# resibots/limbo

Measured on AMD Instinct MI355X. Metric: GP compute()+log_lik evaluations/sec at N=4096 D=6 fp64, higher is better.
Workload: dtype f64

## Files before the change

### limbo_amd/csrc/gemm.hip

```cpp
#include "dev.h"
#include <hip/hip_ext.h>
#include <cstdio>
#include <cstdint>
#include <cstdlib>
#include <map>
#include <mutex>
#include <tuple>
#include <vector>
#include <algorithm>

#ifdef GEMM_TIMING
__device__ long long g_gemm_ts[16];
#define GTS(i) do { if (threadIdx.x == 0 && blockIdx.x == 0 && lwg == (int)blockIdx.x) g_gemm_ts[i] = clock64(); } while (0)
__device__ long long g_gemm64_ts[24];
#define GTS64(i) do { if (threadIdx.x == 0 && blockIdx.x == 0 && lwg == (int)blockIdx.x) g_gemm64_ts[i] = clock64(); } while (0)
#else
#define GTS(i) do { } while (0)
#define GTS64(i) do { } while (0)
#endif
#ifdef GEMM_TIMING
#define GTS64_(i) GTS64(i)
#endif
#include "gemm_glds64.h"
#ifndef GEMM_ABL
#define GEMM_ABL 0
#endif


template <bool KMAJOR, int ROWS, int BK>
struct Stager {
    static constexpr int PER = ROWS * BK / 256;
    static constexpr int STRIDE = ROWS + 16;
    static constexpr int KSTR = BK + 2;
    static constexpr int ELEMS = KMAJOR ? ROWS * KSTR : BK * STRIDE;
    double r[PER];
    template <bool MASKK>
    __device__ __forceinline__ void load(const double* __restrict__ P, int64_t ld, int rl, int kl)
    {
        const int t = threadIdx.x;
        if (!KMAJOR) {
            const int i = t % ROWS, kk0 = t / ROWS;
            constexpr int KS = 256 / ROWS;
            const int ic = i < rl ? i : rl - 1;
#pragma unroll
            for (int q = 0; q < PER; ++q) {
                const int kk = kk0 + KS * q;
                const int kc = kk < kl ? kk : kl - 1;
                const double v = P[ic + (int64_t)kc * ld];
                r[q] = MASKK ? v * (kk < kl ? 1.0 : 0.0) : v;
            }
        }
        else {
            const int kk = t % BK, j0 = t / BK;
            constexpr int JS = 256 / BK;
            const int kc = kk < kl ? kk : kl - 1;
            const double km = kk < kl ? 1.0 : 0.0;
#pragma unroll
            for (int q = 0; q < PER; ++q) {
                const int j = j0 + JS * q;
                const int jc = j < rl ? j : rl - 1;
                const double v = P[kc + (int64_t)jc * ld];
                r[q] = MASKK ? v * km : v;
            }
        }
    }
    __device__ __forceinline__ void store(double* __restrict__ S) const
    {
        const int t = threadIdx.x;
        if (!KMAJOR) {
            const int i = t % ROWS, kk0 = t / ROWS;
            constexpr int KS = 256 / ROWS;
#pragma unroll
            for (int q = 0; q < PER; ++q)
                S[(kk0 + KS * q) * STRIDE + i] = r[q];
        }
        else {
            const int kk = t % BK, j0 = t / BK;
            constexpr int JS = 256 / BK;
#pragma unroll
            for (int q = 0; q < PER; ++q)
                S[(j0 + JS * q) * KSTR + kk] = r[q];
        }
    }
    static __device__ __forceinline__ double at(const double* __restrict__ S, int row, int kq)
    {
        if (!KMAJOR)
            return S[kq * STRIDE + row];
        else
            return S[row * KSTR + kq];
    }
};

template <int TM, int TN, int BKT, int NBUF, bool AK, bool BK, bool BATCH = false>
__global__ __launch_bounds__(256) void k_gemm4(GemmArgs g_)
{
    GemmArgs gb;
    if (BATCH) {
        gb = g_;
        gemm_rebase(gb);
    }
    const GemmArgs& g = BATCH ? gb : g_;
    using SA = Stager<AK, TM, BKT>;
    using SB = Stager<BK, TN, BKT>;
    constexpr int RA = TM / 2 / 16;
    constexpr int RB = TN / 2 / 4;
    __shared__ __attribute__((aligned(16))) double lds[NBUF][SA::ELEMS + SB::ELEMS];
    const int tiles_m = (int)((g.m + TM - 1) / TM);
    const int tiles_n = (int)((g.n + TN - 1) / TN);
    int wg = blockIdx.x;
    {
        const int nwg = gridDim.x;
        const int q = nwg / 8, r = nwg % 8, xcd = wg % 8, idx = wg / 8;
        wg = (xcd < r ? xcd * (q + 1) : r * (q + 1) + (xcd - r) * q) + idx;
    }
    int ti, tj;
    if (g.tri) {
        const int sc = wg / g.fold_len;
        int rr = wg % g.fold_len;
        const int t0 = first_live_tile<TM, TN>(g, sc), c0 = tiles_m - t0;
        if (rr < c0) {
            tj = sc;
            ti = t0 + rr;
        }
        else {
            tj = tiles_n - 1 - sc;
            const int t1 = first_live_tile<TM, TN>(g, tj);
            rr -= c0;
            if (tj == sc || rr >= tiles_m - t1)
                return;
            ti = t1 + rr;
        }
    }
    else {
        ti = wg % tiles_m;
        tj = wg / tiles_m;
    }
    const int64_t row0 = (int64_t)ti * TM, col0 = (int64_t)tj * TN;
    int64_t kbeg = 0;
    if (g.ktri) {
        kbeg = (row0 > col0 ? row0 : col0);
        kbeg -= kbeg % BKT;
    }
    const int64_t kend = g.k;

    const int lane = threadIdx.x & 63;
    const int wave = threadIdx.x >> 6;
    const int wm = (wave & 1) * (TM / 2), wn = (wave >> 1) * (TN / 2);
    const int arow = wm + (lane & 15);
    const int bcol = wn + (lane & 3);
    const int kq = lane >> 4;

    const double* Ap = AK ? g.A + kbeg + row0 * g.lda : g.A + row0 + kbeg * g.lda;
    const double* Bp = BK ? g.B + kbeg + col0 * g.ldb : g.B + col0 + kbeg * g.ldb;
    const int64_t a_kstep = AK ? (int64_t)BKT : (int64_t)BKT * g.lda;
    const int64_t b_kstep = BK ? (int64_t)BKT : (int64_t)BKT * g.ldb;
    const int64_t mrows = g.m - row0, ncols = g.n - col0;
    const int mr = (int)(mrows < TM ? mrows : TM), nc = (int)(ncols < TN ? ncols : TN);

    double acc[RA][RB];
#pragma unroll
    for (int a = 0; a < RA; ++a)
#pragma unroll
        for (int b = 0; b < RB; ++b)
            acc[a][b] = 0.0;

    using WT = WaveTileC<RA, RB>;
    double* Cw = g.C + (col0 + wn) * g.ldc + row0 + wm;
    const int rlim = mr - wm < WT::R ? mr - wm : WT::R, clim = nc - wn < WT::CN ? nc - wn : WT::CN;
    const bool live = rlim > 0 && clim > 0;
    constexpr bool CPRE = (NBUF == 1);
    double cv[WT::NIT];
    if (CPRE && live && g.overwrite != 1)
        WT::load(cv, Cw, g.ldc, rlim, clim, lane);

    SA sa;
    SB sb;
    int64_t kleft = kend - kbeg;
    if (kleft > 0) {
        const int kl = (int)(kleft < BKT ? kleft : BKT);
        sa.template load<true>(Ap, g.lda, mr, kl);
        sb.template load<false>(Bp, g.ldb, nc, kl);
        sa.store(lds[0]);
        sb.store(lds[0] + SA::ELEMS);
    }
    __syncthreads();
    int buf = 0;
    for (int64_t k0 = kbeg; k0 < kend; k0 += BKT) {
#if GEMM_ABL != 1
        const bool more = (NBUF == 2) && (k0 + BKT < kend);
#endif
#if GEMM_ABL == 1
        const bool more = false;
#endif
        if (more) {
            Ap += a_kstep;
            Bp += b_kstep;
            const int64_t kleft2 = kend - k0 - BKT;
            const int kl = (int)(kleft2 < BKT ? kleft2 : BKT);
            sa.template load<true>(Ap, g.lda, mr, kl);
            sb.template load<false>(Bp, g.ldb, nc, kl);
        }
        const double* As = lds[buf];
        const double* Bs = lds[buf] + SA::ELEMS;
#pragma unroll
        for (int ks = 0; ks < BKT; ks += 4) {
            double af[RA], bf[RB];
#pragma unroll
            for (int x = 0; x < RA; ++x)
                af[x] = SA::at(As, arow + 16 * x, ks + kq);
#pragma unroll
            for (int x = 0; x < RB; ++x)
                bf[x] = SB::at(Bs, bcol + 4 * x, ks + kq);
#pragma unroll
            for (int n = 0; n < RB; ++n)
#pragma unroll
                for (int m = 0; m < RA; ++m)
#if GEMM_ABL == 2
                    acc[m][n] += af[m] * bf[n] * (ks == 0 && m == 0 && n == 0 ? 1.0 : 0.0);
#else
                    acc[m][n] = mfma4(af[m], bf[n], acc[m][n]);
#endif
        }
        if (NBUF == 2) {
            if (more) {
                sa.store(lds[buf ^ 1]);
                sb.store(lds[buf ^ 1] + SA::ELEMS);
            }
            __syncthreads();
            buf ^= 1;
        }
    }

    static_assert(4 * WT::SCRATCH <= NBUF * (SA::ELEMS + SB::ELEMS), "transposition scratch must fit in the operand stages");
    if (!CPRE && live && g.overwrite != 1)
        WT::load(cv, Cw, g.ldc, rlim, clim, lane);
    if (NBUF == 1)
        __syncthreads();
    if (live)
        WT::store(acc, cv, &lds[0][0] + wave * WT::SCRATCH, Cw, g.ldc, rlim, clim, g.overwrite, lane);
}

template <typename K>
static void launch_k_named(const char* name, K kern_single, K kern_batched, dim3 grid, dim3 block, hipStream_t s, const GemmArgs& g0)
{
    GemmArgs g = g0;
    g.bt = g_batch.bt;
    grid.z = (unsigned)g_batch.G;
    K kern = g.bt ? kern_batched : kern_single;
    if (g.stop_event)
        GPE_LAUNCH_STOP(name, kern, grid, block, 0, s, (hipEvent_t)g.stop_event, g);
    else
        GPE_LAUNCH_NAMED(name, kern, grid, block, 0, s, g);
}
#define launch_k(ks, ...) launch_k_named(#ks, ks, __VA_ARGS__)
template <int TM, int TN, int BKT, int NBUF>
static void launch_tile(hipStream_t s, const GemmArgs& g0)
{
    GemmArgs g = g0;
    const int tiles_m = (int)((g.m + TM - 1) / TM), tiles_n = (int)((g.n + TN - 1) / TN);
    int64_t tiles = (int64_t)tiles_m * tiles_n;
    if (g.tri) {
        int fold = 1;
        const int nsup = (tiles_n + 1) / 2;
        for (int sc = 0; sc < nsup; ++sc) {
            const int t2 = tiles_n - 1 - sc;
            int len = tiles_m - first_live_tile<TM, TN>(g, sc);
            if (t2 != sc)
                len += tiles_m - first_live_tile<TM, TN>(g, t2);
            fold = len > fold ? len : fold;
        }
        g.fold_len = fold;
        tiles = (int64_t)nsup * fold;
    }
    dim3 grid((unsigned)tiles), block(256);
    if (!g.a_kmajor && !g.b_kmajor)
        launch_k(k_gemm4<TM, TN, BKT, NBUF, false, false>, k_gemm4<TM, TN, BKT, NBUF, false, false, true>, grid, block, s, g);
    else if (!g.a_kmajor && g.b_kmajor)
        launch_k(k_gemm4<TM, TN, BKT, NBUF, false, true>, k_gemm4<TM, TN, BKT, NBUF, false, true, true>, grid, block, s, g);
    else if (g.a_kmajor && !g.b_kmajor)
        launch_k(k_gemm4<TM, TN, BKT, NBUF, true, false>, k_gemm4<TM, TN, BKT, NBUF, true, false, true>, grid, block, s, g);
    else
        launch_k(k_gemm4<TM, TN, BKT, NBUF, true, true>, k_gemm4<TM, TN, BKT, NBUF, true, true, true>, grid, block, s, g);
}


template <int TM, int TN, int WM, int WN, int BKT, int NST, int EPC = 0, int MINB = 1, bool BATCH = false>
__global__ __launch_bounds__(WM* WN * 64, MINB) void k_gemm_glds(GemmArgs g_)
{
    GemmArgs gb;
    if (BATCH) {
        gb = g_;
        gemm_rebase(gb);
    }
    const GemmArgs& g = BATCH ? gb : g_;
    static_assert(TM == 128 && TN == 128, "one k-row of an operand tile = one 1 KiB glds instruction");
    constexpr int NWV = WM * WN;
    constexpr int SA = TM + 16, SB = TN + 16;
    constexpr int STAGE = BKT * (SA + SB);
    constexpr int RA = TM / WM / 16, RB = TN / WN / 4;
    constexpr int LPW = 2 * BKT / NWV;
    __shared__ __attribute__((aligned(16))) double lds[NST * STAGE];

    const int tiles_m = (int)((g.m + TM - 1) / TM);
    const int tiles_n = (int)((g.n + TN - 1) / TN);
    if (g.rhs_rows > 0)
        gemm_rhs_rows<64 * NWV, MINB == 1>(g, g.rhs_rows, (int)gridDim.x, lds);
    for (int lwg = blockIdx.x; lwg < g.total; lwg += gridDim.x) {
    int wg = lwg;
    {
        const int nwg = g.total;
        const int q = nwg / 8, r = nwg % 8, xcd = wg % 8, idx = wg / 8;
        wg = (xcd < r ? xcd * (q + 1) : r * (q + 1) + (xcd - r) * q) + idx;
    }
    int ti, tj;
    if (g.tile_map) {
        const int pk = g.tile_map[lwg];
        if (pk < 0)
            continue;
        ti = pk & 0xffff;
        tj = pk >> 16;
    }
    else if (g.tri) {
        const int sc = wg / g.fold_len;
        int rr = wg % g.fold_len;
        const int t0 = first_live_tile<TM, TN>(g, sc), c0 = tiles_m - t0;
        if (rr < c0) {
            tj = sc;
            ti = t0 + rr;
        }
        else {
            tj = tiles_n - 1 - sc;
            const int t1 = first_live_tile<TM, TN>(g, tj);
            rr -= c0;
            if (tj == sc || rr >= tiles_m - t1)
                continue;
            ti = t1 + rr;
        }
    }
    else {
        ti = wg % tiles_m;
        tj = wg / tiles_m;
    }
    const int64_t row0 = (int64_t)ti * TM, col0 = (int64_t)tj * TN;
    const int64_t mrows = g.m - row0, ncols = g.n - col0;
    const int mr = (int)(mrows < TM ? mrows : TM), nc = (int)(ncols < TN ? ncols : TN);

    const int lane = threadIdx.x & 63;
    const int wave = __builtin_amdgcn_readfirstlane(threadIdx.x >> 6);
    const int wm = (wave % WM) * (TM / WM), wn = (wave / WM) * (TN / WN);
    const int arow = wm + (lane & 15), bcol = wn + (lane & 3), kq = lane >> 4;

    int ra = 2 * lane, rb = 2 * lane;
    {
        const int ma = (mr - 1) & ~1, mb = (nc - 1) & ~1;
        ra = ra < ma ? ra : ma;
        rb = rb < mb ? rb : mb;
    }
    const int64_t kbeg = g.ktri ? (row0 > col0 ? row0 : col0) : 0;
    const double* pa = g.A + row0 + ra + ((int64_t)wave + kbeg) * g.lda;
    const double* pb = g.B + col0 + rb + ((int64_t)wave + kbeg) * g.ldb;
    const int64_t astep = (int64_t)NWV * g.lda, bstep = (int64_t)NWV * g.ldb;

    auto issue = [&](int stage) {
        double* sa = lds + stage * STAGE + wave * SA;
        double* sb = lds + stage * STAGE + BKT * SA + wave * SB;
#pragma unroll
        for (int q = 0; q < BKT / NWV; ++q) {
            __builtin_amdgcn_global_load_lds(pa, (lds_void_t*)(sa + q * NWV * SA), 16, 0, 0);
            __builtin_amdgcn_global_load_lds(pb, (lds_void_t*)(sb + q * NWV * SB), 16, 0, 0);
            pa += astep;
            pb += bstep;
        }
    };

    double acc[RA][RB];
#pragma unroll
    for (int a = 0; a < RA; ++a)
#pragma unroll
        for (int b = 0; b < RB; ++b)
            acc[a][b] = 0.0;

    const int nk = (int)((g.k - kbeg) / BKT);
    GTS(0);
    issue(0);
    for (int t = 0; t < nk; ++t) {
        const int st = t % NST;
        if (t + 1 < nk) {
            issue((t + 1) % NST);
            asm volatile("s_waitcnt vmcnt(%0)" ::"n"(LPW) : "memory");
        }
        else
            asm volatile("s_waitcnt vmcnt(0)" ::: "memory");
        __builtin_amdgcn_s_barrier();
        if (t == 0)
            GTS(1);
        if (t == 1)
            GTS(2);
        if (t == 2)
            GTS(3);
        const double* As = lds + st * STAGE;
        const double* Bs = As + BKT * SA;
#pragma unroll
        for (int ks = 0; ks < BKT; ks += 4) {
            double af[RA], bf[RB];
#pragma unroll
            for (int x = 0; x < RA; ++x)
                af[x] = As[(ks + kq) * SA + arow + 16 * x];
#pragma unroll
            for (int x = 0; x < RB; ++x)
                bf[x] = Bs[(ks + kq) * SB + bcol + 4 * x];
#pragma unroll
            for (int n = 0; n < RB; ++n)
#pragma unroll
                for (int m = 0; m < RA; ++m)
                    acc[m][n] = mfma4(af[m], bf[n], acc[m][n]);
        }
        if (t == 1)
            GTS(6);
        asm volatile("s_waitcnt lgkmcnt(0)" ::: "memory");
        __builtin_amdgcn_s_barrier();
        if (t == 1)
            GTS(7);
    }
    GTS(4);

    {
        using WT = WaveTileC<RA, RB>;
        constexpr int SCR = EPC > 0 ? WT::SCRATCH / EPC : WT::SCRATCH;
        static_assert(NWV * SCR <= NST * STAGE, "transposition scratch must fit in the operand stages");
        double* Cw = g.C + (col0 + wn) * g.ldc + row0 + wm;
        const int rlim = mr - wm < WT::R ? mr - wm : WT::R, clim = nc - wn < WT::CN ? nc - wn : WT::CN;
        if (rlim > 0 && clim > 0) {
            if constexpr (EPC > 0)
                WT::template rmw_chunked<EPC>(acc, lds + wave * SCR, Cw, g.ldc, rlim, clim, g.overwrite, lane);
            else {
                double cv[WT::NIT];
                if (g.overwrite != 1)
                    WT::load(cv, Cw, g.ldc, rlim, clim, lane);
                WT::store(acc, cv, lds + wave * WT::SCRATCH, Cw, g.ldc, rlim, clim, g.overwrite, lane);
            }
        }
    }
    __syncthreads();
    GTS(5);
    }
}
#ifdef GEMM_TIMING
void dump_gemm_timing()
{
    {
        long long q[24];
        (void)hipMemcpyFromSymbol(q, HIP_SYMBOL(g_gemm64_ts), sizeof(q));
        printf("k_gemm_glds64 WG0 first tile, cycles: start->k-tile 0 begins %lld | k-tiles:", q[1] - q[0]);
        for (int t = 1; t < 16; ++t)
            printf(" %lld", q[1 + t] - q[t]);
        printf(" %lld | epilogue %lld | total %lld\n", q[17] - q[16], q[18] - q[17], q[18] - q[0]);
    }
    long long h[16];
    (void)hipMemcpyFromSymbol(h, HIP_SYMBOL(g_gemm_ts), sizeof(h));
    printf("k_gemm_glds WG0 first tile, cycles: prologue (first stage landed) %lld | k-tile 0 %lld | k-tile 1 %lld (mfma part %lld, closing barrier %lld) | whole k loop %lld | epilogue %lld | total %lld\n",
           h[1] - h[0], h[2] - h[1], h[3] - h[2], h[6] - h[2], h[7] - h[6], h[4] - h[1], h[5] - h[4], h[5] - h[0]);
    printf("  epilogue: issue 32 loads %lld | loads complete %lld | issue 32 stores %lld | stores complete %lld | tail %lld\n", h[8] - h[4],
           h[9] - h[8], h[10] - h[9], h[11] - h[10], h[5] - h[11]);
}
#endif

template <int BKT, int NST, int MINB, int NWV, bool BATCH = false>
__global__ __launch_bounds__(64 * NWV, MINB) void k_gemm_glds64(GemmArgs g_)
{
    GemmArgs gb;
    if (BATCH) {
        gb = g_;
        gemm_rebase(gb);
    }
    const GemmArgs& g = BATCH ? gb : g_;
    __shared__ __attribute__((aligned(16))) double lds[NST * Glds64Shape<BKT>::STAGE];
    gemm_glds64_body<BKT, NST, NWV>(g, lds, (int)blockIdx.x, (int)gridDim.x, false);
}

static void launch_glds64(hipStream_t s, const GemmArgs& g0)
{
    constexpr int TM = 64, TN = 64;
    GemmArgs g = g0;
    const int tiles_m = (int)((g.m + TM - 1) / TM), tiles_n = (int)((g.n + TN - 1) / TN);
    int64_t tiles = (int64_t)tiles_m * tiles_n;
    if (g.tri) {
        int fold = 1;
        const int nsup = (tiles_n + 1) / 2;
        for (int sc = 0; sc < nsup; ++sc) {
            const int t2 = tiles_n - 1 - sc;
            int len = tiles_m - first_live_tile<TM, TN>(g, sc);
            if (t2 != sc)
                len += tiles_m - first_live_tile<TM, TN>(g, t2);
            fold = len > fold ? len : fold;
        }
        g.fold_len = fold;
        tiles = (int64_t)nsup * fold;
    }
    g.total = (int)tiles;
    if ((int64_t)g.total * g_batch.G > 256)
        launch_k(k_gemm_glds64<16, 4, 2, 4>, k_gemm_glds64<16, 4, 2, 4, true>, dim3((unsigned)tiles), dim3(256), s, g);
    else
        launch_k(k_gemm_glds64<16, 4, 1, 8>, k_gemm_glds64<16, 4, 1, 8, true>, dim3((unsigned)tiles), dim3(512), s, g);
}

static bool glds_ok(const GemmArgs& g)
{
    return !g.a_kmajor && !g.b_kmajor && !g.ktri && g.k >= 32 && g.k % 32 == 0 && (g.lda % 2) == 0 && (g.ldb % 2) == 0
        && ((uintptr_t)g.A % 16) == 0 && ((uintptr_t)g.B % 16) == 0;
}

#define TRI_BAND 8
struct TriMapKey {
    int dev, tiles_m, tiles_n;
    int64_t off;
    bool operator<(const TriMapKey& o) const
    {
        return std::tie(dev, tiles_m, tiles_n, off) < std::tie(o.dev, o.tiles_m, o.tiles_n, o.off);
    }
};
static int tri_tile_map_host(const GemmArgs& g, std::vector<int>& tab)
{
    constexpr int TM = 128, TN = 128;
    const int tiles_m = (int)((g.m + TM - 1) / TM), tiles_n = (int)((g.n + TN - 1) / TN);
    std::vector<int> first(tiles_n);
    for (int tj = 0; tj < tiles_n; ++tj)
        first[tj] = first_live_tile<TM, TN>(g, tj);
    std::vector<int> seq;
    for (int r0 = 0; r0 < tiles_m; r0 += TRI_BAND) {
        const int r1 = std::min(tiles_m, r0 + TRI_BAND);
        for (int tj = 0; tj < tiles_n; ++tj)
            for (int ti = std::max(r0, first[tj]); ti < r1; ++ti)
                seq.push_back(ti | (tj << 16));
    }
    const int T = (int)seq.size(), q = T / 8, r = T % 8, slots = q + (r ? 1 : 0);
    tab.assign((size_t)slots * 8, -1);
    int pos = 0;
    for (int x = 0; x < 8; ++x) {
        const int len = q + (x < r ? 1 : 0);
        for (int i = 0; i < len; ++i)
            tab[(size_t)i * 8 + x] = seq[pos + i];
        pos += len;
    }
    return (int)tab.size();
}
int debug_tri_tile_map(int64_t m, int64_t n, int64_t grow0, int64_t gcol0, int* out, int cap)
{
    GemmArgs g{};
    g.m = m;
    g.n = n;
    g.tri = 1;
    g.grow0 = grow0;
    g.gcol0 = gcol0;
    std::vector<int> tab;
    const int len = tri_tile_map_host(g, tab);
    for (int i = 0; i < len && i < cap; ++i)
        out[i] = tab[i];
    return len;
}
static const int* tri_tile_map(const GemmArgs& g, int* total)
{
    static std::mutex mu;
    static std::map<TriMapKey, std::pair<int*, int>> cache;
    int dev = 0;
    (void)hipGetDevice(&dev);
    const TriMapKey key{dev, (int)((g.m + 127) / 128), (int)((g.n + 127) / 128), g.gcol0 - g.grow0};
    std::lock_guard<std::mutex> lk(mu);
    auto it = cache.find(key);
    if (it == cache.end()) {
        std::vector<int> tab;
        const int len = tri_tile_map_host(g, tab);
        int* d = nullptr;
        if (hipMalloc(&d, sizeof(int) * (size_t)len) != hipSuccess)
            return nullptr;
        if (hipMemcpy(d, tab.data(), sizeof(int) * (size_t)len, hipMemcpyHostToDevice) != hipSuccess) {
            (void)hipFree(d);
            return nullptr;
        }
        it = cache.emplace(key, std::make_pair(d, len)).first;
    }
    *total = it->second.second;
    return it->second.first;
}

static void launch_glds128(hipStream_t s, const GemmArgs& g0)
{
    constexpr int TM = 128, TN = 128;
    GemmArgs g = g0;
    const int tiles_m = (int)((g.m + TM - 1) / TM), tiles_n = (int)((g.n + TN - 1) / TN);
    int64_t tiles = (int64_t)tiles_m * tiles_n;
    g.tile_map = nullptr;
    int mapped = 0;
    if (g.tri && !g_batch.bt && tiles_m < 65536 && tiles_n < 32768)
        g.tile_map = tri_tile_map(g, &mapped);
    if (g.tile_map)
        tiles = mapped;
    else if (g.tri) {
        int fold = 1;
        const int nsup = (tiles_n + 1) / 2;
        for (int sc = 0; sc < nsup; ++sc) {
            const int t2 = tiles_n - 1 - sc;
            int len = tiles_m - first_live_tile<TM, TN>(g, sc);
            if (t2 != sc)
                len += tiles_m - first_live_tile<TM, TN>(g, t2);
            fold = len > fold ? len : fold;
        }
        g.fold_len = fold;
        tiles = (int64_t)nsup * fold;
    }
    g.total = (int)tiles;
    const bool two_per_cu = (int64_t)g.total * g_batch.G > 256;
    if (two_per_cu)
        launch_k(k_gemm_glds<128, 128, 2, 4, 16, 2, 4, 2>, k_gemm_glds<128, 128, 2, 4, 16, 2, 4, 2, true>, dim3((unsigned)tiles), dim3(512), s, g);
    else
        launch_k(k_gemm_glds<128, 128, 2, 4, 32, 2>, k_gemm_glds<128, 128, 2, 4, 32, 2, 0, 1, true>, dim3((unsigned)tiles), dim3(512), s, g);
}

template <int BKT, int NST, int EPC, int MINB>
__global__ __launch_bounds__(512, MINB) void k_gemm_items(const GemmItem* __restrict__ items, const int32_t* __restrict__ bin_start,
                                                          int64_t ld, const BatchTab* __restrict__ bt, int* __restrict__ counters, int nslots,
                                                          int64_t pstride)
{
    constexpr int TM = 128, TN = 128, WM = 2, WN = 4, NWV = WM * WN;
    constexpr int SA = TM + 16, SB = TN + 16;
    constexpr int STAGE = BKT * (SA + SB);
    constexpr int RA = TM / WM / 16, RB = TN / WN / 4;
    constexpr int LPW = 2 * BKT / NWV;
    __shared__ __attribute__((aligned(16))) double lds[NST * STAGE];
    __shared__ int s_last;
    const int lane = threadIdx.x & 63;
    const int wave = __builtin_amdgcn_readfirstlane(threadIdx.x >> 6);
    const int wm = (wave % WM) * (TM / WM), wn = (wave / WM) * (TN / WN);
    const int arow = wm + (lane & 15), bcol = wn + (lane & 3), kq = lane >> 4;
    const int i0 = bin_start[blockIdx.x], i1 = bin_start[blockIdx.x + 1];
    const int64_t step = (int64_t)NWV * ld;
    for (int it = i0; it < i1; ++it) {
        GemmItem item = items[it];
        if (bt) {
            item.A = bt_rebase(bt, (int)blockIdx.z, item.A);
            item.B = bt_rebase(bt, (int)blockIdx.z, item.B);
            item.C = bt_rebase(bt, (int)blockIdx.z, item.C);
            if (item.T)
                item.T = bt_rebase(bt, (int)blockIdx.z, item.T);
            if (item.nch > 1) {
                item.D = bt_rebase(bt, (int)blockIdx.z, item.D);
                item.P1 = bt_rebase(bt, (int)blockIdx.z, item.P1);
            }
        }
        const int mr = (item.flags >> 8) & 255, nc = (item.flags >> 16) & 255;
        int ra = 2 * lane, rb = 2 * lane;
        {
            const int ma = (mr - 1) & ~1, mb = (nc - 1) & ~1;
            ra = ra < ma ? ra : ma;
            rb = rb < mb ? rb : mb;
        }
        const double* pa = item.A + ra + (int64_t)wave * ld;
        const double* pb = item.B + rb + (int64_t)wave * ld;
        auto issue = [&](int stage) {
            double* sa = lds + stage * STAGE + wave * SA;
            double* sb = lds + stage * STAGE + BKT * SA + wave * SB;
#pragma unroll
            for (int q = 0; q < BKT / NWV; ++q) {
                __builtin_amdgcn_global_load_lds(pa, (lds_void_t*)(sa + q * NWV * SA), 16, 0, 0);
                __builtin_amdgcn_global_load_lds(pb, (lds_void_t*)(sb + q * NWV * SB), 16, 0, 0);
                pa += step;
                pb += step;
            }
        };
        double acc[RA][RB];
#pragma unroll
        for (int a = 0; a < RA; ++a)
#pragma unroll
            for (int b = 0; b < RB; ++b)
                acc[a][b] = 0.0;
        const int nk = item.k / BKT;
        issue(0);
        for (int t = 0; t < nk; ++t) {
            const int st = t % NST;
            if (t + 1 < nk) {
                issue((t + 1) % NST);
                asm volatile("s_waitcnt vmcnt(%0)" ::"n"(LPW) : "memory");
            }
            else
                asm volatile("s_waitcnt vmcnt(0)" ::: "memory");
            __builtin_amdgcn_s_barrier();
            const double* As = lds + st * STAGE;
            const double* Bs = As + BKT * SA;
#pragma unroll
            for (int ks = 0; ks < BKT; ks += 4) {
                double af[RA], bf[RB];
#pragma unroll
                for (int x = 0; x < RA; ++x)
                    af[x] = As[(ks + kq) * SA + arow + 16 * x];
#pragma unroll
                for (int x = 0; x < RB; ++x)
                    bf[x] = Bs[(ks + kq) * SB + bcol + 4 * x];
#pragma unroll
                for (int n = 0; n < RB; ++n)
#pragma unroll
                    for (int m = 0; m < RA; ++m)
                        acc[m][n] = mfma4(af[m], bf[n], acc[m][n]);
            }
            asm volatile("s_waitcnt lgkmcnt(0)" ::: "memory");
            __builtin_amdgcn_s_barrier();
        }
        if (item.flags & 1) {
#pragma unroll
            for (int a = 0; a < RA; ++a)
#pragma unroll
                for (int b = 0; b < RB; ++b)
                    acc[a][b] = -acc[a][b];
        }
        {
            using WT = WaveTileC<RA, RB>;
            constexpr int SCR = WT::SCRATCH / EPC;
            static_assert(NWV * SCR <= NST * STAGE, "transposition scratch must fit in the operand stages");
            const int rlim = mr - wm < WT::R ? mr - wm : WT::R, clim = nc - wn < WT::CN ? nc - wn : WT::CN;
            double* const Tw = item.T ? item.T + wn + (int64_t)wm * ld : nullptr;
            const bool cut = item.nch > 1;
            if (rlim > 0 && clim > 0)
                WT::template store_item<EPC>(acc, lds + wave * SCR, item.C + (int64_t)wn * ld + wm, cut ? nullptr : Tw, ld, rlim, clim, cut, lane);
            if (cut) {
                asm volatile("s_waitcnt vmcnt(0)" ::: "memory");
                __syncthreads();
                if (threadIdx.x == 0)
                    s_last = (__hip_atomic_fetch_add(counters + item.slot + (int)blockIdx.z * nslots, 1, __ATOMIC_RELAXED, __HIP_MEMORY_SCOPE_AGENT) + 1)
                            % item.nch
                        == 0;
                __syncthreads();
                if (s_last && rlim > 0 && clim > 0)
                    WT::template fold_item<EPC>(lds + wave * SCR, item.D + (int64_t)wn * ld + wm, item.P1 + (int64_t)wn * ld + wm, pstride,
                                                item.nch - 1, Tw, ld, rlim, clim, lane);
            }
        }
        __syncthreads();
    }
}

template <int BKT, int NST, int NWV>
__global__ __launch_bounds__(64 * NWV, 4) void k_gemm_items64(const GemmItem* __restrict__ items, const int32_t* __restrict__ bin_start,
                                                               int64_t ld, const BatchTab* __restrict__ bt, int* __restrict__ counters, int nslots,
                                                               int64_t pstride)
{
    static_assert(NWV == 8, "2 x 4 waves of 32 x 16");
    constexpr int PAIR = 144, OPER = (BKT / 2) * PAIR, STAGE = 2 * OPER;
    constexpr int RA = 2, RB = 64 / (NWV / 2) / 4;
    constexpr int LPW = 2 * (BKT / 2) / NWV;
    __shared__ __attribute__((aligned(16))) double lds[NST * STAGE];
    __shared__ int s_last;
    const int lane = threadIdx.x & 63;
    const int wave = __builtin_amdgcn_readfirstlane(threadIdx.x >> 6);
    const int wm = (wave & 1) * 32, wn = (wave >> 1) * (4 * RB);
    const int arow = wm + (lane & 15), bcol = wn + (lane & 3);
    const int kq = lane >> 4, kperm = ((kq & 1) << 1) | (kq >> 1);
    const int r2 = 2 * (lane & 31), khalf = lane >> 5;
    const int i0 = bin_start[blockIdx.x], i1 = bin_start[blockIdx.x + 1];
    const int64_t step8 = (int64_t)(2 * NWV) * ld;
    for (int it = i0; it < i1; ++it) {
        GemmItem item = items[it];
        if (bt) {
            item.A = bt_rebase(bt, (int)blockIdx.z, item.A);
            item.B = bt_rebase(bt, (int)blockIdx.z, item.B);
            item.C = bt_rebase(bt, (int)blockIdx.z, item.C);
            if (item.T)
                item.T = bt_rebase(bt, (int)blockIdx.z, item.T);
            if (item.nch > 1) {
                item.D = bt_rebase(bt, (int)blockIdx.z, item.D);
                item.P1 = bt_rebase(bt, (int)blockIdx.z, item.P1);
            }
        }
        const int mr = (item.flags >> 8) & 255, nc = (item.flags >> 16) & 255;
        const int ma = (mr - 1) & ~1, mb = (nc - 1) & ~1;
        const double* pa = item.A + (r2 < ma ? r2 : ma) + (int64_t)(2 * wave + khalf) * ld;
        const double* pb = item.B + (r2 < mb ? r2 : mb) + (int64_t)(2 * wave + khalf) * ld;
        auto issue = [&](int stage) {
            double* sa = lds + stage * STAGE + wave * PAIR;
            double* sb = sa + OPER;
#pragma unroll
            for (int q = 0; q < BKT / 2 / NWV; ++q) {
                __builtin_amdgcn_global_load_lds(pa, (lds_void_t*)(sa + NWV * q * PAIR), 16, 0, 0);
                __builtin_amdgcn_global_load_lds(pb, (lds_void_t*)(sb + NWV * q * PAIR), 16, 0, 0);
                pa += step8;
                pb += step8;
            }
        };
        double acc[RA][RB];
#pragma unroll
        for (int a = 0; a < RA; ++a)
#pragma unroll
            for (int b = 0; b < RB; ++b)
                acc[a][b] = 0.0;
        const int nk = item.k / BKT;
        for (int t = 0; t < NST - 1 && t < nk; ++t)
            issue(t);
        for (int t = 0; t < nk; ++t) {
            const int st = t % NST;
            if (t + NST - 1 < nk)
                issue((t + NST - 1) % NST);
            const int ahead = nk - 1 - t < NST - 1 ? nk - 1 - t : NST - 1;
            if (ahead >= 3)
                asm volatile("s_waitcnt vmcnt(%0)" ::"n"(3 * LPW) : "memory");
            else if (ahead == 2)
                asm volatile("s_waitcnt vmcnt(%0)" ::"n"(2 * LPW) : "memory");
            else if (ahead == 1)
                asm volatile("s_waitcnt vmcnt(%0)" ::"n"(1 * LPW) : "memory");
            else
                asm volatile("s_waitcnt vmcnt(0)" ::: "memory");
            __builtin_amdgcn_s_barrier();
            const double* As = lds + st * STAGE;
            const double* Bs = As + OPER;
#pragma unroll
            for (int ks = 0; ks < BKT; ks += 4) {
                const int k = ks + kperm;
                const int off = (k >> 1) * PAIR + (k & 1) * 64;
                double af[RA], bf[RB];
#pragma unroll
                for (int x = 0; x < RA; ++x)
                    af[x] = As[off + arow + 16 * x];
#pragma unroll
                for (int x = 0; x < RB; ++x)
                    bf[x] = Bs[off + bcol + 4 * x];
#pragma unroll
                for (int n = 0; n < RB; ++n)
#pragma unroll
                    for (int m = 0; m < RA; ++m)
                        acc[m][n] = mfma4(af[m], bf[n], acc[m][n]);
            }
            asm volatile("s_waitcnt lgkmcnt(0)" ::: "memory");
            __builtin_amdgcn_s_barrier();
        }
        if (item.flags & 1) {
#pragma unroll
            for (int a = 0; a < RA; ++a)
#pragma unroll
                for (int b = 0; b < RB; ++b)
                    acc[a][b] = -acc[a][b];
        }
        {
            using WT = WaveTileC<RA, RB>;
            static_assert(NWV * WT::SCRATCH <= NST * STAGE, "transposition scratch must fit in the operand stages");
            const int rlim = mr - wm < WT::R ? mr - wm : WT::R, clim = nc - wn < WT::CN ? nc - wn : WT::CN;
            double* const Tw = item.T ? item.T + wn + (int64_t)wm * ld : nullptr;
            const bool cut = item.nch > 1;
            if (rlim > 0 && clim > 0)
                WT::template store_item<1>(acc, lds + wave * WT::SCRATCH, item.C + (int64_t)wn * ld + wm, cut ? nullptr : Tw, ld, rlim, clim, cut, lane);
            if (cut) {
                asm volatile("s_waitcnt vmcnt(0)" ::: "memory");
                __syncthreads();
                if (threadIdx.x == 0)
                    s_last = (__hip_atomic_fetch_add(counters + item.slot + (int)blockIdx.z * nslots, 1, __ATOMIC_RELAXED, __HIP_MEMORY_SCOPE_AGENT) + 1)
                            % item.nch
                        == 0;
                __syncthreads();
                if (s_last && rlim > 0 && clim > 0)
                    WT::template fold_item<1>(lds + wave * WT::SCRATCH, item.D + (int64_t)wn * ld + wm, item.P1 + (int64_t)wn * ld + wm, pstride,
                                              item.nch - 1, Tw, ld, rlim, clim, lane);
            }
        }
        __syncthreads();
    }
}

void launch_gemm_items(hipStream_t s, const GemmItem* items, const int32_t* bin_start, int nbins, int64_t ld, int tile, int* counters, int nslots,
                       int64_t pstride)
{
    if (nbins > 0 && tile == 64) {
        GPE_LAUNCH_NAMED("k_gemm_items64", (k_gemm_items64<16, 4, 8>), dim3((unsigned)nbins, 1, (unsigned)g_batch.G), dim3(512), 0, s, items,
                         bin_start, ld, g_batch.bt, counters, nslots, pstride);
        return;
    }

    if (nbins <= 0)
        return;
    GPE_LAUNCH_NAMED("k_gemm_items", (k_gemm_items<16, 2, 4, 4>), dim3((unsigned)nbins, 1, (unsigned)g_batch.G), dim3(512), 0, s, items, bin_start,
                     ld, g_batch.bt, counters, nslots, pstride);
}

static int64_t live_tiles(const GemmArgs& g, int TM, int TN)
{
    const int64_t tm = (g.m + TM - 1) / TM, tn = (g.n + TN - 1) / TN;
    if (!g.tri)
        return tm * tn;
    int64_t cnt = 0;
    for (int64_t tj = 0; tj < tn; ++tj) {
        int64_t need = g.gcol0 + tj * TN - g.grow0 - (TM - 1);
        int64_t ti0 = need <= 0 ? 0 : (need + TM - 1) / TM;
        if (ti0 < tm)
            cnt += tm - ti0;
    }
    return cnt;
}

static void launch_gemm_sub_impl(hipStream_t s, const GemmArgs& g);
void launch_gemm_sub(hipStream_t s, const GemmArgs& g0)
{
    if (g0.m <= 0 || g0.n <= 0)
        return;
    if (g0.k <= 0 && !g0.overwrite)
        return;
    if (g0.rhs_rows > 0) {
        GemmArgs q = g0;
        q.m = g0.m - g0.rhs_rows;
        q.rhs_rows = 0;
        bool fma = false;
        if (q.m > 0 && !q.overwrite && glds_ok(q) && g_batch.G == 1) {
            auto crosses = [&](int T, int64_t round) { return live_tiles(q, T, T) <= round && live_tiles(g0, T, T) > round; };
            fma = crosses(128, 256) || (live_tiles(g0, 128, 128) < 200 && (crosses(64, 512) || crosses(64, 256)));
        }
        if (fma) {
            q.rhs_rows = g0.rhs_rows;
            launch_gemm_sub_impl(s, q);
        }
        else {
            q = g0;
            q.rhs_rows = 0;
            launch_gemm_sub_impl(s, q);
        }
        return;
    }
    launch_gemm_sub_impl(s, g0);
}

static void launch_gemm_sub_impl(hipStream_t s, const GemmArgs& g)
{
    int tile = g.tile;
    if (tile != 128 && tile != 64 && tile != 32) {
        const int64_t GB = g_batch.G;
        const int64_t t128_min = 200;
        if (glds_ok(g) && GB * live_tiles(g, 128, 128) >= t128_min)
            tile = 128;
        else if (glds_ok(g) && !g.ktri && GB * live_tiles(g, 64, 64) >= 96)
            tile = 64;
        else if (GB * live_tiles(g, 64, 64) >= 512)
            tile = 64;
        else
            tile = 32;
    }
    if (g.rhs_rows > 0) {
        const bool direct = glds_ok(g) && (tile == 128 || (tile == 64 && !g.ktri));
        if (!direct) {
            GemmArgs q = g;
            q.m += q.rhs_rows;
            q.rhs_rows = 0;
            launch_gemm_sub_impl(s, q);
            return;
        }
    }
    if (tile == 128 && glds_ok(g))
        launch_glds128(s, g);
    else if (tile == 128)
        launch_tile<128, 128, 32, 2>(s, g);
    else if (tile == 64 && glds_ok(g) && !g.ktri)
        launch_glds64(s, g);
    else if (tile == 64)
        launch_tile<64, 64, 32, 2>(s, g);
    else if (g.k <= 64 && !g.ktri)
        launch_tile<32, 64, 64, 1>(s, g);
    else
        launch_tile<32, 64, 32, 2>(s, g);
}

double gemm_flops(const GemmArgs& g)
{
    double m = (double)g.m, n = (double)g.n, k = (double)g.k;
    if (g.ktri)
        return n * n * n / 3.0;
    if (g.tri) {
        double off = (double)(g.grow0 - g.gcol0);
        double cnt = 0.0;
        double jfull = off < n ? off : n;
        cnt += jfull * m;
        double rest = n - jfull;
        if (rest > 0) {
            double first = m, last = m - (rest - 1);
            if (last < 0) {
                rest = m + 1;
                last = 0;
            }
            cnt += 0.5 * (first + last) * rest;
        }
        return 2.0 * cnt * k;
    }
    return 2.0 * m * n * k;
}
```

Measured before the change: 946.9.

## Stagger half the waves' MFMA k-steps across the barrier in glds GEMM

Adds a STAG template parameter to the glds128 GEMM kernel. With it, the upper half of the waves defers their last k-slice fragments past the stage barrier and computes them while the next stage loads, and those waves also get raised s_setprio. Setting 25 (S=1, behind-mode, priority, lead sched_barrier) becomes the default for the one-block-per-CU shape. The aim is to desynchronise the waves so LDS reads and MFMA issue from different waves overlap instead of all waves stalling at the barrier together. The cost is extra registers for the carried fragments, a second code path, and a debug entry point for testing stagger variants.

```diff
diff --git a/limbo_amd/csrc/gemm.hip b/limbo_amd/csrc/gemm.hip
--- a/limbo_amd/csrc/gemm.hip
+++ b/limbo_amd/csrc/gemm.hip
@@ -6,6 +6,7 @@
 #include <map>
 #include <mutex>
 #include <tuple>
+#include <type_traits>
 #include <vector>
 #include <algorithm>
 
@@ -283,8 +284,7 @@
         launch_k(k_gemm4<TM, TN, BKT, NBUF, true, true>, k_gemm4<TM, TN, BKT, NBUF, true, true, true>, grid, block, s, g);
 }
 
-
-template <int TM, int TN, int WM, int WN, int BKT, int NST, int EPC = 0, int MINB = 1, bool BATCH = false>
+template <int TM, int TN, int WM, int WN, int BKT, int NST, int EPC = 0, int MINB = 1, bool BATCH = false, int STAG = 0>
 __global__ __launch_bounds__(WM* WN * 64, MINB) void k_gemm_glds(GemmArgs g_)
 {
     GemmArgs gb;
@@ -380,9 +380,60 @@
         for (int b = 0; b < RB; ++b)
             acc[a][b] = 0.0;
 
+    constexpr int S = STAG & 3;
+    constexpr bool SBEHIND = (STAG & 4) != 0;
+    static_assert(S < BKT / 4 && (S > 0 || (STAG & 4) == 0), "stagger");
+    constexpr bool LEADPIN = (STAG & 16) != 0;
+    const bool lag = S > 0 && wave >= NWV / 2;
+    auto frags = [&](const double* As, const double* Bs, int ks, double (&af)[RA], double (&bf)[RB]) {
+#pragma unroll
+        for (int x = 0; x < RA; ++x)
+            af[x] = As[(ks + kq) * SA + arow + 16 * x];
+#pragma unroll
+        for (int x = 0; x < RB; ++x)
+            bf[x] = Bs[(ks + kq) * SB + bcol + 4 * x];
+    };
+    auto mults = [&](const double (&af)[RA], const double (&bf)[RB]) {
+#pragma unroll
+        for (int n = 0; n < RB; ++n)
+#pragma unroll
+            for (int m = 0; m < RA; ++m)
+                acc[m][n] = mfma4(af[m], bf[n], acc[m][n]);
+    };
     const int nk = (int)((g.k - kbeg) / BKT);
+    if constexpr ((STAG & 8) != 0) {
+        if (wave >= NWV / 2)
+            __builtin_amdgcn_s_setprio(1);
+    }
     GTS(0);
     issue(0);
+    auto kloop = [&](auto role) {
+    constexpr bool LAG = decltype(role)::value;
+    double caf[LAG ? S : 1][RA], cbf[LAG ? S : 1][RB];
+#pragma unroll
+    for (int s = 0; s < (LAG ? S : 1); ++s) {
+#pragma unroll
+        for (int x = 0; x < RA; ++x)
+            caf[s][x] = 0.0;
+#pragma unroll
+        for (int x = 0; x < RB; ++x)
+            cbf[s][x] = 0.0;
+    }
+    auto carried = [&]() {
+        __builtin_amdgcn_sched_barrier(0);
+#pragma unroll
+        for (int s = 0; s < (LAG ? S : 0); ++s) {
+#pragma unroll
+            for (int x = 0; x < RA; ++x)
+                asm volatile("" : "+v"(caf[s][x]));
+#pragma unroll
+            for (int x = 0; x < RB; ++x)
+                asm volatile("" : "+v"(cbf[s][x]));
+        }
+#pragma unroll
+        for (int s = 0; s < (LAG ? S : 0); ++s)
+            mults(caf[s], cbf[s]);
+    };
     for (int t = 0; t < nk; ++t) {
         const int st = t % NST;
         if (t + 1 < nk) {
@@ -400,6 +451,25 @@
             GTS(3);
         const double* As = lds + st * STAGE;
         const double* Bs = As + BKT * SA;
+        if constexpr (LAG) {
+            if constexpr (SBEHIND) {
+                double af[RA], bf[RB];
+                frags(As, Bs, 0, af, bf);
+                if (t > 0)
+                    carried();
+                mults(af, bf);
+            }
+#pragma unroll
+            for (int ks = SBEHIND ? 4 : 0; ks < BKT - 4 * S; ks += 4) {
+                double af[RA], bf[RB];
+                frags(As, Bs, ks, af, bf);
+                mults(af, bf);
+            }
+#pragma unroll
+            for (int s = 0; s < S; ++s)
+                frags(As, Bs, BKT - 4 * S + 4 * s, caf[s], cbf[s]);
+        }
+        else {
 #pragma unroll
         for (int ks = 0; ks < BKT; ks += 4) {
             double af[RA], bf[RB];
@@ -414,6 +484,9 @@
 #pragma unroll
                 for (int m = 0; m < RA; ++m)
                     acc[m][n] = mfma4(af[m], bf[n], acc[m][n]);
+        }
+        if constexpr (LEADPIN)
+            __builtin_amdgcn_sched_barrier(0);
         }
         if (t == 1)
             GTS(6);
@@ -421,7 +494,26 @@
         __builtin_amdgcn_s_barrier();
         if (t == 1)
             GTS(7);
-    }
+        if constexpr (LAG && !SBEHIND) {
+            carried();
+            __builtin_amdgcn_sched_barrier(0);
+        }
+    }
+    if constexpr (LAG && SBEHIND) {
+        if (nk > 0)
+            carried();
+    }
+    };
+    if constexpr (S > 0) {
+        if (lag)
+            kloop(std::true_type{});
+        else
+            kloop(std::false_type{});
+    }
+    else
+        kloop(std::false_type{});
+    if constexpr ((STAG & 8) != 0)
+        __builtin_amdgcn_s_setprio(0);
     GTS(4);
 
     {
@@ -583,7 +675,10 @@
     return it->second.first;
 }
 
-static void launch_glds128(hipStream_t s, const GemmArgs& g0)
+#define GLDS_STAG_ONE 25
+#define GLDS_STAG_TWO 0
+#define GLDS_STAG_TWO_HOOK 1
+static void launch_glds128(hipStream_t s, const GemmArgs& g0, int shape = -1, int stag = -1, int grid_cap = 0)
 {
     constexpr int TM = 128, TN = 128;
     GemmArgs g = g0;
@@ -609,11 +704,107 @@
         tiles = (int64_t)nsup * fold;
     }
     g.total = (int)tiles;
-    const bool two_per_cu = (int64_t)g.total * g_batch.G > 256;
-    if (two_per_cu)
-        launch_k(k_gemm_glds<128, 128, 2, 4, 16, 2, 4, 2>, k_gemm_glds<128, 128, 2, 4, 16, 2, 4, 2, true>, dim3((unsigned)tiles), dim3(512), s, g);
-    else
-        launch_k(k_gemm_glds<128, 128, 2, 4, 32, 2>, k_gemm_glds<128, 128, 2, 4, 32, 2, 0, 1, true>, dim3((unsigned)tiles), dim3(512), s, g);
+    const bool two_per_cu = shape < 0 ? (int64_t)g.total * g_batch.G > 256 : shape == 1;
+    const dim3 grid((unsigned)(grid_cap > 0 && grid_cap < tiles ? grid_cap : tiles)), block(512);
+#define GLDS_ONE(ST) launch_k_named("k_gemm_glds<128", k_gemm_glds<128, 128, 2, 4, 32, 2, 0, 1, false, ST>, k_gemm_glds<128, 128, 2, 4, 32, 2, 0, 1, true>, grid, block, s, g)
+#define GLDS_TWO(ST) launch_k_named("k_gemm_glds<128", k_gemm_glds<128, 128, 2, 4, 16, 2, 4, 2, false, ST>, k_gemm_glds<128, 128, 2, 4, 16, 2, 4, 2, true>, grid, block, s, g)
+    const int on = two_per_cu ? (GLDS_STAG_TWO ? GLDS_STAG_TWO : GLDS_STAG_TWO_HOOK) : GLDS_STAG_ONE;
+    const int code = stag < 0 ? (two_per_cu ? GLDS_STAG_TWO : GLDS_STAG_ONE) : stag == 0 ? 0 : stag == 1 ? on : stag - 16;
+    if (two_per_cu) {
+        switch (code) {
+        case 0: GLDS_TWO(0); break;
+        case GLDS_STAG_TWO_HOOK: GLDS_TWO(GLDS_STAG_TWO_HOOK); break;
+#ifdef GEMM_STAG_STUDY
+        case 5: GLDS_TWO(5); break;
+        case 8: GLDS_TWO(8); break;
+        case 9: GLDS_TWO(9); break;
+#endif
+        default: fprintf(stderr, "launch_glds128: no such stagger %d\n", code); break;
+        }
+    }
+    else {
+        switch (code) {
+        case 0: GLDS_ONE(0); break;
+        case GLDS_STAG_ONE: GLDS_ONE(GLDS_STAG_ONE); break;
+#ifdef GEMM_STAG_STUDY
+        case 1: GLDS_ONE(1); break;
+        case 2: GLDS_ONE(2); break;
+        case 5: GLDS_ONE(5); break;
+        case 6: GLDS_ONE(6); break;
+        case 8: GLDS_ONE(8); break;
+        case 9: GLDS_ONE(9); break;
+        case 10: GLDS_ONE(10); break;
+        case 13: GLDS_ONE(13); break;
+        case 14: GLDS_ONE(14); break;
+        case 16: GLDS_ONE(16); break;
+        case 17: GLDS_ONE(17); break;
+        case 18: GLDS_ONE(18); break;
+        case 21: GLDS_ONE(21); break;
+        case 24: GLDS_ONE(24); break;
+        case 26: GLDS_ONE(26); break;
+        case 29: GLDS_ONE(29); break;
+#endif
+        default: fprintf(stderr, "launch_glds128: no such stagger %d\n", code); break;
+        }
+    }
+#undef GLDS_ONE
+#undef GLDS_TWO
+}
+
+extern "C" int gpe_debug_gemm_stagger(const double* A, const double* B, double* C, int64_t m, int64_t n, int64_t k, int tri, int64_t grow0,
+                                      int64_t gcol0, int ktri, int overwrite, int rhs_rows, int shape, int stag, int grid_cap)
+{
+    if (!A || !B || !C || m <= 0 || n <= 0 || k < 32 || k % 32 || m > (1 << 20) || n > (1 << 20) || k > (1 << 20) || rhs_rows < 0 || rhs_rows > 64
+        || overwrite < 0 || overwrite > 2 || (rhs_rows > 0 && overwrite) || (shape != 0 && shape != 1) || stag < 0 || grid_cap < 0)
+        return -1;
+#ifndef GEMM_STAG_STUDY
+    if (stag > 1)
+        return -1;
+#endif
+    if (ktri && (tri || k != n || m != n || rhs_rows))
+        return -1;
+    const int64_t mt = m + rhs_rows, lda = (mt + 3) & ~(int64_t)1, ldb = (n + 3) & ~(int64_t)1;
+    double *dA = nullptr, *dB = nullptr, *dC = nullptr;
+    int rc = -2;
+    hipStream_t s = nullptr;
+    do {
+        if (hipMalloc(&dA, sizeof(double) * lda * k) != hipSuccess || hipMalloc(&dB, sizeof(double) * ldb * k) != hipSuccess
+            || hipMalloc(&dC, sizeof(double) * lda * n) != hipSuccess)
+            break;
+        if (hipMemset(dA, 0, sizeof(double) * lda * k) != hipSuccess || hipMemset(dB, 0, sizeof(double) * ldb * k) != hipSuccess
+            || hipMemset(dC, 0, sizeof(double) * lda * n) != hipSuccess)
+            break;
+        if (hipMemcpy2D(dA, sizeof(double) * lda, A, sizeof(double) * mt, sizeof(double) * mt, k, hipMemcpyHostToDevice) != hipSuccess
+            || hipMemcpy2D(dB, sizeof(double) * ldb, B, sizeof(double) * n, sizeof(double) * n, k, hipMemcpyHostToDevice) != hipSuccess
+            || hipMemcpy2D(dC, sizeof(double) * lda, C, sizeof(double) * mt, sizeof(double) * mt, n, hipMemcpyHostToDevice) != hipSuccess)
+            break;
+        GemmArgs g{};
+        g.C = dC;
+        g.ldc = lda;
+        g.A = dA;
+        g.lda = lda;
+        g.B = dB;
+        g.ldb = ldb;
+        g.m = m;
+        g.n = n;
+        g.k = k;
+        g.tri = tri ? 1 : 0;
+        g.grow0 = grow0;
+        g.gcol0 = gcol0;
+        g.ktri = ktri ? 1 : 0;
+        g.overwrite = overwrite;
+        g.rhs_rows = rhs_rows;
+        launch_glds128(s, g, shape, stag, grid_cap);
+        if (hipGetLastError() != hipSuccess || hipStreamSynchronize(s) != hipSuccess)
+            break;
+        if (hipMemcpy2D(C, sizeof(double) * mt, dC, sizeof(double) * lda, sizeof(double) * mt, n, hipMemcpyDeviceToHost) != hipSuccess)
+            break;
+        rc = 0;
+    } while (0);
+    (void)hipFree(dA);
+    (void)hipFree(dB);
+    (void)hipFree(dC);
+    return rc;
 }
 
 template <int BKT, int NST, int EPC, int MINB>
```

After: 950.6 (median of 6 runs). About the same (+0.4%).
